# daviszhen/plan

Hardware: NVIDIA B200
Metric: tpch_q1_q6_q3_lineitem_rows_per_s (higher is better)
Workload: dtype int64 fixed-point (128-bit merge)

## Files before the change

### plan_b200/csrc/join.cu

```cuda
#include <algorithm>

#include <cub/device/device_scan.cuh>

#include "hostdec.hpp"
#include "join.cuh"
#include "exchange.cuh"
#include "leftcount.cuh"
#include "pipeline.hpp"

namespace pg {

namespace {

struct BaseCol { int slot = -1, col = -1; };

struct Stage {
    int src_slot = -1;
    std::vector<Range> ranges;
    bool has_probe = false;
    int probe_mode = 0;
    bool existence_only = false;
    int probe_key_col = -1;
    int probe_stage = -1;
    int ins_key_col = -1;
// ... 13 lines not shown
    bool no_table = false;
    i64 dup_keys = 0;
    bool bitmap_only() const { return jt.bitmap && !payload_needed && (dup_keys == 0 || existence_only); }
};

static u64 next_pow2(u64 x)
{
    u64 p = 1;
    while (p < x) p <<= 1;
    return p;
}

static TypedCol typed(const pg_table *t, int col)
{
    TypedCol c;
    c.p = t->cols[(size_t)col].d_data;
    c.width = t->cols[(size_t)col].phys_width();
    c.base = t->cols[(size_t)col].base;
    c.valid = t->cols[(size_t)col].has_nulls ? t->cols[(size_t)col].d_valid : nullptr;
    return c;
}

}

struct JoinAggPipeline : Pipeline {
    pg_plan *plan = nullptr;
    std::vector<std::unique_ptr<Stage>> stages;
    int src_slot = -1;
    std::vector<Range> ranges;
    int probe_key_col = -1;
    GroupSpec gs{};
    int nparts = 0;
    BaseCol part_col[GT_MAXKEYPARTS];
    int part_type[GT_MAXKEYPARTS] = {0, 0, 0};
    std::vector<AggExpr> aggs;
    std::vector<int> agg_scale;
    std::vector<int> agg_plane;
    bool no_join = false;
    int top_probe_mode = 0;
    int hav_plane = -1;
    i64 hav_lo = INT64_MIN, hav_hi = INT64_MAX;
    i64 group_hint = 0;
    i64 key_min = 0;
    u64 key_domain = 0;
    bool key_sorted = false;
    bool device_only = false;
    i64 dev_ngroups = 0;
    std::vector<Stage::Extra> extras;
    bool fd_mode = false;
    struct FdOut { int kind, slot, col, via_key_col, via_stage; };
    std::vector<FdOut> fd;
    int fd_stage = -1;
    int star_anchor = -1;
    bool star = false;
    int main_stage = -1;
    struct HRef { int origin = 0, col = -1; };
    struct HLookup { int nkey = 1; HRef key[2]; int stage = -1; };
    struct HPart { HRef v; int fn = 0; i64 lo = 0; int n = 1; int type = 0; };
    struct HTerm { int nfac = 0; HRef fac[3]; i64 fc[3] = {0, 0, 0}; int fs[3] = {1, 1, 1}; i64 mul = 1; };
    std::vector<HLookup> lookups;
    std::vector<int> origin_slot;
    std::vector<HPart> sparts;
    std::vector<HTerm> sterms;
    int star_ngroups = 0, star_scale = 0;
    i128 star_worst = 0;
    int xl = -1;
    std::vector<int> xcols;
    int x_term_mask[STAR_MAXTERM] = {0, 0};
    int x_fac_col[STAR_MAXTERM][3] = {{0, 0, 0}, {0, 0, 0}};
    DevBuf d_xb_rec, d_xb_dest, d_xb_send, d_xb_recv, d_xp_rec, d_xp_dest, d_xp_send, d_xp_recv;
    i64 xb_recv_rows = 0;
    EventPair ev_xb, ev_xp;
    i64 x_sent_rows = 0, x_sent_bytes = 0;
    DevBuf d_star, d_star_all;
    PinBuf h_star;
    Stage &top_stage_ref() { return *stages[(size_t)(main_stage >= 0 ? main_stage : (int)stages.size() - 1)]; }
    DevBuf d_edges, d_dense;
    int dense_passes = 0;
    std::vector<std::pair<int, int>> outs;
    std::vector<int> group_out_type;
    i64 algorithmic_bytes = 0, main_bytes = 0;
    DevBuf d_counters, d_gt, d_overflow, d_out_klo, d_out_khi, d_out_acc;
    u64 gt_cap = 0;
    i64 out_cap = 0;
    EventPair ev_all, ev_main;
    bool shuffle = false;
    bool gather_ranks = false;
    DevBuf d_g_klo, d_g_khi, d_g_acc, d_g_cnt;
    PinBuf h_out;
    static constexpr int SG_CAP = 256;
    DevBuf d_sg;
    PinBuf h_sg;
    bool has_topk = false;
    TopkKey topk_key{};
    i64 topk_limit = -1;
    DevBuf d_hist, d_cand_klo, d_cand_khi, d_cand_acc, d_tstate;
    PinBuf h_hist;
    i64 cand_cap = 0;

    int topk_preselect(i64 *ngroups, pg_result *res)
    {
        cudaStream_t st = ctx().stream;
        i64 n = *ngroups, k = topk_limit;
        if (k < 0 || n <= k) return PG_OK;
        if (k == 0) { *ngroups = 0; return PG_OK; }
        const int planes = gs.nacc + 1 + (int)fd.size();
// ... 127 lines not shown
    {
        unsigned long long h[8];
        PG_CUDA(cudaMemcpyAsync(h, d_counters.p, 64, cudaMemcpyDeviceToHost, ctx().stream));
        PG_CUDA(cudaStreamSynchronize(ctx().stream));
        memcpy(out2, h, 32);
        for (int idx = 0; idx < 2; idx++)
            if (((deferred_stats >> idx) & 1u) && cur_res) {
                cur_res->stats.aux[2 + 2 * idx] = (i64)h[4 + 2 * idx];
                cur_res->stats.aux[3 + 2 * idx] = (i64)h[5 + 2 * idx];
            }
        return PG_OK;
    }

    static int grid_rows(i64 nrows)
    {
        i64 g = (nrows + 255) / 256;
        i64 cap = (i64)ctx().prop.multiProcessorCount * 8;
        if (g > cap) g = cap;
        return (int)std::max<i64>(g, 1);
    }

    DevBuf d_hits, d_hit_count;
    static constexpr i64 HIT_CHUNK = (i64)1 << 30;

    static bool two_phase_ok(const PipeParams &pp, const pg_table *t, bool ins_sink)
    {
        bool any_valid = pp.probe_key.valid != nullptr || (ins_sink && pp.ins_key.valid != nullptr);
        for (int k = 0; k < pp.npred; k++) any_valid = any_valid || pp.pred[k].col.valid != nullptr;
        return (pp.has_probe ? pp.probe.bitmap != nullptr : ins_sink) && pp.nlike == 0 && pp.npred <= 1 && (pp.npred == 0 || !pp.pred[0].is_set) && !any_valid && t->nrows < ((i64)1 << 32) &&
               !getenv("PG_JOIN_GENERIC");
    }

    int launch_filter(PipeParams &pp, i64 lo, i64 hi)
    {
        cudaStream_t st = ctx().stream;
        if (!d_hit_count.p) PG_TRY(d_hit_count.alloc(8));
        size_t need = (size_t)std::max<i64>(hi - lo, 1) * 4;
        if (d_hits.bytes < need) PG_TRY(d_hits.alloc(need));
        PG_CUDA(cudaMemsetAsync(d_hit_count.p, 0, 8, st));
        pp.row_begin = lo;
        pp.row_end = hi;
        pp.hits = d_hits.as<unsigned>();
        pp.hit_count = d_hit_count.as<unsigned long long>();
        if (try_staged_filter(pp, lo, hi) == PG_OK) return PG_OK;
        i64 ntiles = (hi - lo + SA_TILE - 1) / SA_TILE;
        int grid = (int)std::max<i64>(std::min<i64>(ntiles, (i64)ctx().prop.multiProcessorCount * 8), 1);
        if (pp.npred == 1) filter_hits_kernel<true, 1><<<grid, SA_THREADS, 0, st>>>(pp);
        else filter_hits_kernel<false, 1><<<grid, SA_THREADS, 0, st>>>(pp);
        PG_CUDA(cudaGetLastError());
        return PG_OK;
    }

    bool staged_filter_used = false;
    int try_staged_filter(const PipeParams &pp, i64 lo, i64 hi)
    {
        if (getenv("PG_NO_STAGED") && atoi(getenv("PG_NO_STAGED"))) return PG_EUNSUPPORTED;
        if (hi <= lo || (lo & 15) != 0 || pp.npred > 1) return PG_EUNSUPPORTED;
        const TypedCol &kc = pp.probe_key;
        if (!kc.p || kc.width > 4 || kc.valid) return PG_EUNSUPPORTED;
        FilterSParams fp{};
        fp.bitmap = pp.has_probe ? pp.probe.bitmap : nullptr;
        if (pp.has_probe && !fp.bitmap) return PG_EUNSUPPORTED;
        fp.anti = pp.probe_mode == 2 ? 1 : 0;
        auto stored_span = [](const TypedCol &c, i64 *tmin, i64 *tmax) {
            if (c.width == 4) { *tmin = INT32_MIN; *tmax = INT32_MAX; }
            else { *tmin = 0; *tmax = c.width == 2 ? 0xffff : 0xff; }
        };
        if (fp.bitmap) {
            if (pp.probe.domain > 0xffffffffULL) return PG_EUNSUPPORTED;
            i64 tmin, tmax;
            stored_span(kc, &tmin, &tmax);
            const i128 delta = (i128)kc.base - (i128)pp.probe.bm_min;
            const i128 omin = (i128)tmin + delta, omax = (i128)tmax + delta;
            if (omax >= ((i128)1 << 32) || omin <= (i128)pp.probe.domain - ((i128)1 << 32)) return PG_EUNSUPPORTED;
            fp.kdelta = (unsigned)(u64)(i64)delta;
            fp.dom = (unsigned)pp.probe.domain;
        }
        fp.p_lo = 0; fp.p_span = 0xffffffffu;
        fp.st.ncol = 0;
        fp.rpw[0] = 0; fp.roff[0] = 0;
        int pi = -1;
        if (pp.npred == 1) {
            const TypedCol &pc = pp.pred[0].col;
            if (pp.pred[0].is_set || pc.width > 4 || pc.valid) return PG_EUNSUPPORTED;
            i64 tmin, tmax;
            stored_span(pc, &tmin, &tmax);
            i128 a = (i128)pp.pred[0].lo - pc.base, b = (i128)pp.pred[0].hi - pc.base;
            if (a < tmin) a = tmin;
            if (b > tmax) b = tmax;
            if (pp.pred[0].lo > pp.pred[0].hi || a > b) return PG_EUNSUPPORTED;
            fp.p_lo = (unsigned)(int32_t)(i64)a;
            fp.p_span = (unsigned)(u64)(i64)(b - a);
            pi = fp.st.ncol;
            fp.st.src[pi] = (const char *)pc.p + lo * pc.width;
            fp.st.pw[pi] = pc.width;
            fp.st.ncol++;
        }
        int ki = -1;
        if (pi >= 0 && fp.st.src[pi] == (const char *)kc.p + lo * kc.width) ki = pi;
        else {
            ki = fp.st.ncol;
            fp.st.src[ki] = (const char *)kc.p + lo * kc.width;
            fp.st.pw[ki] = kc.width;
            fp.st.ncol++;
        }
        const int qpt = 2;
        const int tile_rows = ST_CONS_WARPS * 128 * qpt;
        stage_layout(&fp.st, tile_rows);
        if (pi >= 0) { fp.rpw[0] = fp.st.pw[pi]; fp.roff[0] = fp.st.off[pi]; }
        fp.rpw[1] = fp.st.pw[ki]; fp.roff[1] = fp.st.off[ki];
        fp.st.nstage = getenv("PG_NSTAGE") ? atoi(getenv("PG_NSTAGE")) : 4;
        fp.row_begin = lo;
        fp.nloc = hi - lo;
        fp.hits = pp.hits;
        fp.hit_count = pp.hit_count;
        fp.counters = pp.counters;
        typedef void (*FK)(const FilterSParams);
        FK k;
        if (const char *m = getenv("PG_STAGED_FILTER_MASK")) {
            const int cls = (fp.rpw[0] == 2 && fp.rpw[1] == 4) ? 1 : (fp.rpw[0] == 0 && fp.rpw[1] == 4) ? 2 : fp.rpw[0] == 0 ? 4 : 8;
            if (!(atoi(m) & cls)) return PG_EUNSUPPORTED;
        }
        if (fp.rpw[0] == 2 && fp.rpw[1] == 4) k = filter_hits_staged_kernel<2, 4, 2>;
        else if (fp.rpw[0] == 0 && fp.rpw[1] == 4) k = filter_hits_staged_kernel<0, 4, 2>;
        else if (fp.rpw[0] == 0) k = filter_hits_staged_kernel<0, -1, 2>;
        else k = filter_hits_staged_kernel<-1, -1, 2>;
        const size_t smem = (size_t)ST_HDR + (size_t)fp.st.nstage * fp.st.stage_bytes;
        PG_CUDA(cudaFuncSetAttribute((const void *)k, cudaFuncAttributeMaxDynamicSharedMemorySize, (int)smem));
        int per_sm = 1;
        cudaOccupancyMaxActiveBlocksPerMultiprocessor(&per_sm, (const void *)k, ST_THREADS, smem);
        const i64 ntiles = (fp.nloc + tile_rows - 1) / tile_rows;
        const int grid = (int)std::max<i64>(1, std::min<i64>(ntiles, (i64)ctx().prop.multiProcessorCount * std::max(per_sm, 1)));
        k<<<grid, ST_THREADS, smem, ctx().stream>>>(fp);
        PG_CUDA(cudaGetLastError());
        staged_filter_used = true;
        return PG_OK;
    }

    template <int SINK>
    int launch_sink(const PipeParams &pp)
    {
        hits_sink_kernel<SINK><<<ctx().prop.multiProcessorCount * 8, 256, 0, ctx().stream>>>(pp);
        PG_CUDA(cudaGetLastError());
        return PG_OK;
    }

    template <int SINK>
    int launch_pipe(const PipeParams &pp, const pg_table *t)
    {
        pipeline_kernel<SINK><<<grid_rows(pp.pipe_hi > 0 ? pp.pipe_hi - pp.pipe_lo : t->nrows), 256, 0, ctx().stream>>>(pp);
        PG_CUDA(cudaGetLastError());
        return PG_OK;
    }

    int prepare_table(Stage &s, i64 nbuild, const Column &keycol)
    {
        cudaStream_t st = ctx().stream;
        u64 nb = next_pow2((u64)std::max<i64>((nbuild * 2 + HT_BUCKET - 1) / HT_BUCKET, 16));
        if (nbuild > s.capacity_rows || !s.d_slots.p) {
            PG_TRY(s.d_slots.alloc(nb * HT_BUCKET * sizeof(longlong2)));
            s.capacity_rows = (i64)(nb * HT_BUCKET / 2);
        } else {
            nb = next_pow2((u64)std::max<i64>((nbuild * 2 + HT_BUCKET - 1) / HT_BUCKET, 16));
        }
        PG_CUDA(cudaMemsetAsync(s.d_slots.p, 0x80, nb * HT_BUCKET * sizeof(longlong2), st));
        s.jt.slots = s.d_slots.as<longlong2>();
        s.jt.bucket_mask = nb - 1;
        {
            i128 dom = (i128)keycol.vmax - (i128)keycol.vmin + 1;
            int lg = 0;
            while (((u64)1 << lg) < nb) lg++;
            bool asc = keycol.stats_ok && keycol.adjacent_descents * 100 <= std::max<i64>(nbuild, 1) && dom > 0 && dom <= ((i128)1 << 34) && lg <= 29;
            if (getenv("PG_JOIN_ORDER_PRESERVING")) asc = asc && atoi(getenv("PG_JOIN_ORDER_PRESERVING")) != 0;
            if (s.ins_key_col2 >= 0) asc = false;
            s.jt.order_preserving = asc ? 1 : 0;
            s.jt.log2buckets = lg;
            s.jt.domain = dom > 0 ? (u64)dom : 1;
        }
        s.jt.rank_prefix = nullptr;
        s.jt.rank_payload = nullptr;
        s.jt.rank_identity = 0;
        s.rank_index = false;
        s.jt.bitmap = nullptr;
        s.jt.bm_min = keycol.vmin;
        s.jt.bm_max = keycol.vmax;
        i128 domain = (i128)keycol.vmax - (i128)keycol.vmin + 1;
        if (keycol.stats_ok && domain > 0 && domain <= ((i128)1 << 32) && s.ins_key_col2 < 0) {
// ... 629 lines not shown
                const AggExpr &a = aggs[(size_t)o.second];
                col.width = a.width;
                col.scale = a.scale;
                if (a.fn == PG_AGG_AVG && a.ltype == PG_LT_DOUBLE) {
                    col.type = PG_T_FLOAT64;
                    col.data.resize(live.size() * 8);
                    double *d = (double *)col.data.data();
                    for (size_t i = 0; i < live.size(); i++) {
                        const i128 v = sums[(size_t)live[i]];
                        if (v >= ((i128)1 << 53) || v <= -((i128)1 << 53)) PG_FAIL(PG_EOVERFLOW, "avg(INT): sum not exact in float64");
                        d[i] = (double)(i64)v / (double)cnts[(size_t)live[i]];
                    }
                } else if (a.fn == PG_AGG_AVG) {
                    col.type = PG_T_DECIMAL128;
                    col.data.resize(live.size() * sizeof(pg_decimal));
                    pg_decimal *d = (pg_decimal *)col.data.data();
                    for (size_t i = 0; i < live.size(); i++) {
                        HDec sd, nd, qd;
                        if (!hd_from_i128(sums[(size_t)live[i]], star_scale, &sd) || !hd_from_i128((i128)cnts[(size_t)live[i]], 0, &nd) || !hd_quo(sd, nd, &qd))
                            PG_FAIL(PG_EOVERFLOW, "avg: decimal division failed");
                        d[i].coef = qd.coef;
                        d[i].scale = qd.scale;
                        d[i].neg = qd.neg ? 1u : 0u;
                    }
                } else if (a.fn == PG_AGG_COUNT || a.ltype == PG_LT_HUGEINT) {
                    col.type = PG_T_HUGEINT;
                    col.data.resize(live.size() * sizeof(pg_hugeint));
                    pg_hugeint *d = (pg_hugeint *)col.data.data();
                    for (size_t i = 0; i < live.size(); i++) {
                        const i128 v = a.fn == PG_AGG_COUNT ? (i128)cnts[(size_t)live[i]] : sums[(size_t)live[i]];
                        d[i].lower = (u64)v;
                        d[i].upper = (i64)(v >> 64);
                    }
                } else {
                    col.type = PG_T_DECIMAL128;
                    col.data.resize(live.size() * sizeof(pg_decimal));
                    pg_decimal *d = (pg_decimal *)col.data.data();
                    for (size_t i = 0; i < live.size(); i++) {
                        const i128 v = sums[(size_t)live[i]];
                        const u128 m = v < 0 ? (u128)(-v) : (u128)v;
                        if (m >= (u128)10000000000000000000ULL) PG_FAIL(PG_EOVERFLOW, "star join: a group sum needs more than 19 digits");
                        d[i].neg = v < 0;
                        d[i].coef = (u64)m;
                        d[i].scale = star_scale;
                    }
                }
            }
            res->cols.push_back(std::move(col));
        }
        tr.mark("result columns");
        return PG_OK;
    }

    int run(pg_result *res) override
    {
        Context &c = ctx();
        cudaStream_t st = c.stream;
        PG_TRY(ev_all.init());
        PG_TRY(ev_main.init());
        Trace tr("joinagg");
        PG_CUDA(cudaEventRecord(ev_all.a, st));
        res->stats.kernel_launches = 0;
        cur_res = res;
        deferred_stats = 0;
        PG_CUDA(cudaMemsetAsync(d_counters.p, 0, 128, st));
        x_sent_rows = x_sent_bytes = 0;
        for (size_t i = 0; i < stages.size(); i++) {
            if (xl >= 0 && (int)i == lookups[(size_t)xl].stage) { PG_TRY(run_exchange_build(*stages[i], res)); tr.mark("build stage (row exchange)"); continue; }
            PG_TRY(run_build_stage(*stages[i], res, (int)i));
            tr.mark("build stage");
        }
        if (star) return run_star(res, tr);

        const pg_table *t = tab(src_slot);
        PipeParams pp{};
        pp.nrows = t->nrows;
        PG_TRY(fill_preds(pp, ranges, src_slot));
        pp.has_probe = no_join ? 0 : 1;
        if (!no_join) {
            Stage &last = top_stage_ref();
            pp.probe_key = typed(t, probe_key_col);
            pp.probe = last.jt;
            pp.probe_bitmap_only = last.bitmap_only() ? 1 : 0;
            pp.probe_mode = top_probe_mode;
        }
        PG_TRY(fill_extras(pp, extras, src_slot));
        pp.counters = d_counters.as<unsigned long long>();
        pp.gs = gs;
        u64 cap = next_pow2((u64)std::max<i64>((no_join ? group_hint : stages.back()->built_rows) * 2, 1024));
        unsigned long long cnt[4] = {0, 0, 0, 0};
        const bool two_phase = !no_join && two_phase_ok(pp, t, false);
        const bool single_filter = two_phase && t->nrows <= HIT_CHUNK;
        unsigned long long filter_pass = 0;
        if (single_filter) {
            PG_CUDA(cudaMemsetAsync(d_counters.p, 0, 32, st));
            PG_CUDA(cudaEventRecord(ev_main.a, st));
            PG_TRY(launch_filter(pp, 0, t->nrows));
            unsigned long long c0[4];
            PG_TRY(read_counters(c0));
            filter_pass = c0[0];
            const bool exact = pp.probe_bitmap_only || pp.probe_mode != 0 || stages.back()->dup_keys == 0 || stages.back()->unique_key;
            if (exact) cap = next_pow2((u64)std::max<i64>((i64)std::min<unsigned long long>(c0[3], (unsigned long long)cap / 2) * 2, 1024));
            res->stats.kernel_launches += 1;
            tr.mark("probe filter");
        }
        bool one_shape = false;
        if (no_join) {
            bool pred_valid = false;
            for (int k = 0; k < pp.npred; k++) pred_valid = pred_valid || pp.pred[k].col.valid != nullptr;
            one_shape = !pred_valid && gs.nparts == 1 && gs.nacc == 1 && gs.nfac[0] == 1 && pp.npred <= 1 &&
                        (pp.npred == 0 || !pp.pred[0].is_set) && !getenv("PG_GROUP_GENERIC");
        }
        const bool sorted_runs = one_shape && key_sorted && t->nrows > 0 && !(shuffle && c.world > 1) && !getenv("PG_NO_SORTED_RUNS");
        i64 ngroups = 0;
        if (sorted_runs) {
            constexpr int WPB = SA_THREADS / 32;
            const i64 ntiles = (t->nrows + RUN_WTILE - 1) / RUN_WTILE;
            i64 nwarps = std::max<i64>(std::min<i64>(ntiles, (i64)c.prop.multiProcessorCount * 4 * WPB), 1);
            const i64 chunk_tiles = (ntiles + nwarps - 1) / nwarps;
            nwarps = (ntiles + chunk_tiles - 1) / chunk_tiles;
            const i64 grid = (nwarps + WPB - 1) / WPB;
            const i64 nchunks = grid * WPB;
            if (d_edges.bytes < (size_t)nchunks * 2 * sizeof(RunEdge)) PG_TRY(d_edges.alloc((size_t)nchunks * 2 * sizeof(RunEdge)));
            RunEdge *first = d_edges.as<RunEdge>(), *last = first + nchunks;
            i64 want = hav_plane >= 0 ? std::max<i64>(t->nrows / 64, 1 << 16) : std::min<i64>(t->nrows, group_hint * 4);
            for (int attempt = 0;; attempt++) {
                if (want > out_cap) {
                    PG_TRY(d_out_klo.alloc((size_t)want * 8));
                    PG_TRY(d_out_khi.alloc((size_t)want * 8));
                    PG_TRY(d_out_acc.alloc((size_t)want * 8 * (size_t)(gs.nacc + 1)));
                    out_cap = want;
                }
                PG_CUDA(cudaMemsetAsync(d_counters.p, 0, 32, st));
                RunOut ro{d_out_klo.as<i64>(), d_out_khi.as<i64>(), d_out_acc.as<i64>(), out_cap, d_counters.as<unsigned long long>() + 2,
                          hav_plane, hav_lo, hav_hi};
                PG_CUDA(cudaEventRecord(ev_main.a, st));
                if (pp.npred == 1) run_group_kernel<true><<<(int)grid, SA_THREADS, 0, st>>>(pp, ro, first, last, chunk_tiles);
                else run_group_kernel<false><<<(int)grid, SA_THREADS, 0, st>>>(pp, ro, first, last, chunk_tiles);
                PG_CUDA(cudaGetLastError());
                run_fixup_kernel<<<(int)((nchunks + 255) / 256), 256, 0, st>>>(first, last, (int)nchunks, ro);
                PG_CUDA(cudaGetLastError());
                PG_CUDA(cudaEventRecord(ev_main.b, st));
                res->stats.kernel_launches += 2;
                PG_TRY(read_counters(cnt));
                ngroups = (i64)cnt[2];
// ... 294 lines not shown
                PG_CUDA(cudaMemcpyAsync(nh.p, d_out_khi.p, (size_t)ngroups * 8, cudaMemcpyDeviceToDevice, st));
                for (int a = 0; a < planes; a++)
                    PG_CUDA(cudaMemcpyAsync(na.as<i64>() + (size_t)a * (size_t)maxn, d_out_acc.as<i64>() + (size_t)a * (size_t)out_cap,
                                            (size_t)ngroups * 8, cudaMemcpyDeviceToDevice, st));
                PG_CUDA(cudaStreamSynchronize(st));
                std::swap(d_out_klo.p, nk.p); std::swap(d_out_klo.bytes, nk.bytes);
                std::swap(d_out_khi.p, nh.p); std::swap(d_out_khi.bytes, nh.bytes);
                std::swap(d_out_acc.p, na.p); std::swap(d_out_acc.bytes, na.bytes);
                out_cap = maxn;
            }
            size_t seg = (size_t)maxn * 8;
            if (d_g_klo.bytes < seg * (size_t)c.world) {
                PG_TRY(d_g_klo.alloc(seg * (size_t)c.world));
                PG_TRY(d_g_khi.alloc(seg * (size_t)c.world));
                PG_TRY(d_g_acc.alloc(seg * (size_t)c.world * (size_t)planes));
            }
            PG_TRY(comm_allgather(d_out_klo.p, d_g_klo.p, seg, st));
            PG_TRY(comm_allgather(d_out_khi.p, d_g_khi.p, seg, st));
            for (int a = 0; a < planes; a++)
                PG_TRY(comm_allgather(d_out_acc.as<i64>() + (size_t)a * (size_t)out_cap,
                                      (char *)d_g_acc.p + (size_t)a * seg * (size_t)c.world, seg, st));
            PG_TRY(host_arrays(total));
            i64 off = 0;
            for (int r = 0; r < c.world; r++) {
                size_t n = (size_t)counts[(size_t)r];
                if (n) {
                    PG_CUDA(cudaMemcpyAsync(h_klo + off, (char *)d_g_klo.p + seg * (size_t)r, n * 8, cudaMemcpyDeviceToHost, st));
                    PG_CUDA(cudaMemcpyAsync(h_khi + off, (char *)d_g_khi.p + seg * (size_t)r, n * 8, cudaMemcpyDeviceToHost, st));
                    for (int a = 0; a < planes; a++)
                        PG_CUDA(cudaMemcpyAsync(h_acc + (size_t)a * (size_t)total + (size_t)off,
                                                (char *)d_g_acc.p + (size_t)a * seg * (size_t)c.world + seg * (size_t)r, n * 8,
                                                cudaMemcpyDeviceToHost, st));
                }
                off += (i64)n;
            }
            ngroups = total;
        } else {
            PG_TRY(host_arrays(ngroups));
            if (ngroups > 0) {
                PG_CUDA(cudaMemcpyAsync(h_klo, d_out_klo.p, (size_t)ngroups * 8, cudaMemcpyDeviceToHost, st));
                PG_CUDA(cudaMemcpyAsync(h_khi, d_out_khi.p, (size_t)ngroups * 8, cudaMemcpyDeviceToHost, st));
                for (int a = 0; a < planes; a++)
                    PG_CUDA(cudaMemcpyAsync(h_acc + (size_t)a * (size_t)ngroups, d_out_acc.as<i64>() + (size_t)a * (size_t)out_cap,
                                            (size_t)ngroups * 8, cudaMemcpyDeviceToHost, st));
            }
        }
        PG_CUDA(cudaEventRecord(ev_all.b, st));
        PG_CUDA(cudaStreamSynchronize(st));
        tr.mark("gather+d2h");
        res->stats.kernel_ms = ev_all.ms();
        res->stats.main_kernel_ms = ev_main.ms();
        res->stats.rows_scanned = t->nrows;
        res->stats.algorithmic_bytes = algorithmic_bytes;
        res->stats.main_kernel_bytes = main_bytes + (i64)cnt[1] * 32 * (gs.nparts + 2 * gs.nacc);
        res->stats.aux[0] = (i64)cnt[0];
        res->stats.aux[1] = (i64)cnt[1];

        res->nrows = ngroups;
        for (auto &o : outs) {
            ResCol col;
            if (o.first == 0 && fd_mode) {
                const FdOut &fo = fd[(size_t)o.second];
                const Column &cc = tab(fo.slot)->cols[(size_t)fo.col];
                const i64 *src = h_acc + (size_t)(gs.nacc + 1 + o.second) * (size_t)ngroups;
                col.type = cc.type;
                col.width = cc.width;
                col.scale = cc.scale;
                if (cc.type == PG_T_DICT8) col.dict = cc.dict;
                const int w = type_size(cc.type);
                col.data.resize((size_t)ngroups * (size_t)w);
                if (cc.type == PG_T_VARCHAR) {
                    size_t total = 0;
                    for (i64 i = 0; i < ngroups; i++) {
                        if (src[i] < 0 || src[i] + 1 >= (i64)cc.h_off.size()) PG_FAIL(PG_ECUDA, "internal: dependent key row %lld out of range", (long long)src[i]);
                        total += (size_t)(cc.h_off[(size_t)src[i] + 1] - cc.h_off[(size_t)src[i]]);
                    }
                    col.heap.resize(total + 1);
                    pg_string *d = (pg_string *)col.data.data();
                    size_t at = 0;
                    for (i64 i = 0; i < ngroups; i++) {
                        const size_t b = (size_t)cc.h_off[(size_t)src[i]], n = (size_t)cc.h_off[(size_t)src[i] + 1] - b;
                        memcpy(col.heap.data() + at, cc.h_bytes.data() + b, n);
                        d[i].data = col.heap.data() + at;
                        d[i].len = (int64_t)n;
                        at += n;
                    }
                } else {
                    for (i64 i = 0; i < ngroups; i++) {
                        if (w == 8) ((i64 *)col.data.data())[i] = src[i];
                        else if (w == 4) ((int32_t *)col.data.data())[i] = (int32_t)src[i];
                        else col.data[(size_t)i] = (uint8_t)src[i];
                    }
                }
            } else if (o.first == 0) {
                int k = o.second;
                col.type = group_out_type[(size_t)k];
                const int w = type_size(col.type);
                col.data.resize((size_t)ngroups * (size_t)w);
                if (k == 0 && w == 8) {
                    if (ngroups) memcpy(col.data.data(), h_klo, (size_t)ngroups * 8);
                } else if (k == 0) {
                    int32_t *d = (int32_t *)col.data.data();
                    for (i64 i = 0; i < ngroups; i++) d[i] = (int32_t)h_klo[i];
                } else if (w == 4) {
                    int32_t *d = (int32_t *)col.data.data();
                    if (k == 1) for (i64 i = 0; i < ngroups; i++) d[i] = (int32_t)(h_khi[i] >> 32);
                    else for (i64 i = 0; i < ngroups; i++) d[i] = (int32_t)(h_khi[i] & 0xffffffffLL);
// ... 966 lines not shown
            p->shuffle = !(ok && disjoint);
            if (p->fd_mode) {
                if (bt->dist == PG_DIST_REPLICATED) PG_FAIL(PG_EUNSUPPORTED, "dependent group keys over a replicated build table and a sharded probe");
                for (auto &f : p->fd)
                    if (p->tab(f.slot)->cols[(size_t)f.col].type == PG_T_VARCHAR && p->tab(f.slot)->dist != PG_DIST_REPLICATED)
                        PG_FAIL(PG_EUNSUPPORTED, "VARCHAR group key from a sharded table");
                p->shuffle = false;
            }
        }
    }
    if (plan->topk && !plan->topk->order.empty() && !nested && !p->fd_mode) {
        auto o = aggn.outs[(size_t)plan->topk->order[0].first];
        TopkKey tk{};
        tk.desc = plan->topk->order[0].second ? 1 : 0;
        tk.div = 1;
        if (o.first == 0) {
            tk.src = o.second;
        } else {
            if (aggn.aggs[(size_t)o.second].fn == PG_AGG_AVG) goto no_device_topk;
            tk.src = 3;
            tk.plane = p->agg_plane[(size_t)o.second];
            int sc = p->agg_scale[(size_t)o.second];
            for (int i = 2; i < sc; i++) tk.div *= 10;
        }
        p->has_topk = true;
        p->topk_key = tk;
        p->topk_limit = plan->topk->limit;
    }
no_device_topk:
    PG_TRY(p->d_counters.alloc(128));
    PG_TRY(p->d_overflow.alloc(4));
    std::string ex = "JoinAgg[inner hash join chain -> global group table] stages:";
    for (auto &sp : p->stages) {
        char b[256];
        snprintf(b, sizeof b, " build(%s%s key=%s%s%s)", sp->sub ? "aggregate over " : "", p->tab(sp->src_slot)->name.c_str(),
                 p->tab(sp->src_slot)->cols[(size_t)sp->ins_key_col].name.c_str(), sp->has_probe ? " probing previous" : "",
                 sp->extras.empty() ? "" : " +existence tests");
        ex += b;
    }
    if (p->fd_mode) ex += " group-by=build row id (dependent keys fetched per group)";
    char b[320];
    if (p->no_join)
        snprintf(b, sizeof b, "GroupBy[global open-addressing table] scan(%s) kernel=pipeline_kernel<SINK_GROUP> group_keys=%d sums=%d%s%s%s",
                 st->name.c_str(), p->nparts, p->gs.nacc, p->hav_plane >= 0 ? " having" : "",
                 p->key_sorted ? " sorted-run reduce-by-key when the shape allows (run_group_kernel)"
                               : (p->key_domain > 0 && p->key_domain <= ((u64)1 << 28)) ? " dense direct-addressed accumulators in L2-sized key slices when the shape allows (group1_dense_kernel)" : "",
                 p->shuffle ? " exchange=all-to-all(hash-partitioned)" : "");
    else
        snprintf(b, sizeof b, " probe(%s key=%s) kernel=filter_hits_kernel+hits_sink_kernel<SINK_GROUP> group_keys=%d sums=%d%s", st->name.c_str(),
                 st->cols[(size_t)p->probe_key_col].name.c_str(), p->nparts, p->gs.nacc,
                 p->shuffle ? " exchange=all-to-all(hash-partitioned)" : "");
    if (p->no_join) ex = b; else ex += b;
    p->explain = ex;
    *out = std::move(p);
    return PG_OK;
}

}


namespace pg {

namespace {

struct LeftCountPipeline : Pipeline {
    JoinAggPipeline jp;
    int anchor_col = -1;
    int build_slot = -1, build_key_col = -1;
    int arg_col = -1;
    bool null_if_empty = false;
    bool outer = false;
    std::vector<Range> build_ranges;
    std::vector<std::pair<int, int>> outs;
    LcFilter fa{}, fb{};
    DevBuf d_counts, d_cnt, d_hist, d_out_key, d_out_cnt;
    i64 big_cap = 0;
    EventPair ev_all, ev_main;
    i64 main_bytes = 0, algorithmic_bytes = 0;

    int fill(LcFilter &f, const std::vector<Range> &rs, int slot, std::vector<std::string> *desc)
    {
        const pg_table *t = jp.tab(slot);
        const bool bytewise = getenv("PG_LIKE_BYTEWISE") && atoi(getenv("PG_LIKE_BYTEWISE")) != 0;
        f.npred = f.nlike = 0;
        for (auto &r : rs) {
            if (!r.like) {
                if (f.npred >= PIPE_MAXPRED) PG_FAIL(PG_EUNSUPPORTED, "more than %d predicate columns on one scan", PIPE_MAXPRED);
                SrcPred &q = f.pred[f.npred++];
                q.col = typed(t, r.col);
                q.lo = r.lo;
                q.hi = r.hi;
                q.is_set = r.is_set ? 1 : 0;
                memcpy(q.mask, r.set, sizeof q.mask);
                continue;
            }
            const Column &col = t->cols[(size_t)r.col];
            if (!col.d_off) PG_FAIL(PG_EUNSUPPORTED, "string predicate on %s without a device copy of the text", col.name.c_str());
            if (f.nlike >= GEN_MAXLIKE) PG_FAIL(PG_EUNSUPPORTED, "more than %d string predicates on one scan", GEN_MAXLIKE);
            GenLike &l = f.like[f.nlike++];
            memset(&l, 0, sizeof l);
            l.bytes = col.d_bytes;
            l.off = (const i64 *)col.d_off;
            std::vector<std::string> segs;
            if (r.like <= 2 && !bytewise && like_segments(r.pat, &segs)) {
                l.kind = r.like == 1 ? GEN_LIKE_WORDS : GEN_NOTLIKE_WORDS;
                l.plen = (int)segs.size();
// ... 280 lines not shown
```

### plan_b200/csrc/join.cuh

```cuda
#pragma once
#include "common.cuh"
#include "scanagg.cuh"

namespace pg {

constexpr i64 HT_EMPTY = (i64)0x8080808080808080ULL;
constexpr int HT_BUCKET = 4;

__host__ __device__ __forceinline__ u64 mix64(u64 x)
{
    x ^= x >> 33; x *= 0xff51afd7ed558ccdULL; x ^= x >> 33; x *= 0xc4ceb9fe1a85ec53ULL; x ^= x >> 33;
    return x;
}

struct JoinTable {
    longlong2 *slots;
    u64 bucket_mask;
    unsigned *bitmap;
    i64 bm_min, bm_max;
    unsigned long long *dups;
    int order_preserving;
    int log2buckets;
    u64 domain;
    const unsigned *rank_prefix;
// ... 843 lines not shown
        base = __shfl_sync(0xffffffffu, base, 0);
        for (int i = lane; i < nbuf; i += 32) p.hits[base + i] = s_buf[warp][i];
        __syncwarp();
        n_hits += lane == 0 ? (unsigned)nbuf : 0u;
        nbuf = 0;
    }
    int pos = nbuf + incl - c;
#pragma unroll
    for (int q = 0; q < QPT; q++) {
        const unsigned rowid = (unsigned)(p.row_begin + row0) + (unsigned)((warp * QPT + q) * 128 + lane * 4);
#pragma unroll
        for (int j = 0; j < 4; j++)
            if (hitmask & (1u << (4 * q + j))) s_buf[warp][pos++] = rowid + j;
    }
    nbuf += total;
    __syncwarp();
}

template <int WP, int WK, int QPT>
__global__ void __launch_bounds__(ST_THREADS)
filter_hits_staged_kernel(const FilterSParams p)
{
    extern __shared__ __align__(128) unsigned char st_smem[];
    __shared__ unsigned s_buf[ST_CONS_WARPS][512];
    const StageDesc &d = p.st;
    const StageRing ring = stage_ring_init(st_smem, d);
    const i64 ntiles = (p.nloc + d.tile_rows - 1) / d.tile_rows;
    const TileSeq seq = tile_seq(ntiles, 0);
    const int warp = threadIdx.x >> 5, lane = threadIdx.x & 31;
    if (warp == ST_CONS_WARPS) {
        stage_produce(ring, d, seq);
        return;
    }
    StageCursor cur = {0, 0};
    int nbuf = 0;
    unsigned n_pass = 0, n_hits = 0;
    const bool partial = last_tile_is_partial(seq, ntiles, p.nloc, d.tile_rows);
    const int nwhole = (int)seq.count - (partial ? 1 : 0);
    for (int k = 0; k < nwhole; k++)
        filter_tile<WP, WK, QPT, false>(p, ring, cur, warp, lane, seq.first + (i64)k * seq.step, s_buf, nbuf, n_pass, n_hits);
    if (partial) filter_tile<WP, WK, QPT, true>(p, ring, cur, warp, lane, ntiles - 1, s_buf, nbuf, n_pass, n_hits);
    if (nbuf) {
        unsigned long long base = 0;
        if (lane == 0) base = atomicAdd(p.hit_count, (unsigned long long)nbuf);
        base = __shfl_sync(0xffffffffu, base, 0);
        for (int i = lane; i < nbuf; i += 32) p.hits[base + i] = s_buf[warp][i];
        n_hits += lane == 0 ? (unsigned)nbuf : 0u;
    }
    unsigned long long np = (unsigned long long)warp_sum((i64)n_pass), nh = (unsigned long long)warp_sum((i64)n_hits);
    if (lane == 0 && np) atomicAdd(&p.counters[0], np);
    if (lane == 0 && nh) atomicAdd(&p.counters[3], nh);
}

template <int SINK>
__global__ void __launch_bounds__(256)
hits_sink_kernel(const PipeParams p)
{
    const unsigned long long n = *p.hit_count;
    unsigned long long n_join = 0;
    for (unsigned long long i = (unsigned long long)blockIdx.x * blockDim.x + threadIdx.x; i < n; i += (unsigned long long)gridDim.x * blockDim.x) {
        const i64 row = (i64)p.hits[i];
        if (p.nextra && !extras_pass(p, row)) continue;
        auto sink = [&](u64 build_row) {
            n_join++;
            if (SINK == SINK_INSERT) {
                i64 key = load_typed(p.ins_key, row);
                if (p.ins_key2.p) key = (key << 32) | (load_typed(p.ins_key2, row) & 0xffffffffLL);
                jt_insert(p.ins, key, (u64)row);
            } else if (SINK == SINK_BITMAP) {
                u64 off = (u64)(load_typed(p.ins_key, row) - p.ins.bm_min);
                atomicOr(p.ins.bitmap + (off >> 5), 1u << (off & 31));
            } else if (SINK == SINK_GROUP) {
                auto val = [&](const ValRef &r) { return r.from_build == 2 ? (i64)build_row : load_typed(r.col, r.from_build ? (i64)build_row : row); };
                i64 klo = val(p.gs.part[0]);
                i64 khi = 0;
                if (p.gs.nparts > 1) khi = val(p.gs.part[1]) << 32;
                if (p.gs.nparts > 2) khi |= val(p.gs.part[2]) & 0xffffffffLL;
                i64 vals[GT_MAXACC];
                for (int a = 0; a < p.gs.nacc; a++) {
                    i64 x = 1;
                    for (int f = 0; f < p.gs.nfac[a]; f++) x *= p.gs.fc[a][f] + p.gs.fs[a][f] * val(p.gs.fac[a][f]);
                    vals[a] = x;
                }
                gt_update(p.gt, klo, khi, vals);
            }
        };
        if (!p.has_probe || p.probe_bitmap_only || p.probe_mode != 0) sink(0);
        else jt_probe(p.probe, load_typed(p.probe_key, row), sink);
    }
    n_join = (unsigned long long)warp_sum((i64)n_join);
    if ((threadIdx.x & 31) == 0 && n_join) atomicAdd(&p.counters[1], n_join);
}

constexpr int STAR_MAXLOOKUP = 5, STAR_MAXTERM = 2, STAR_MAXPART = 2, STAR_MAXGROUPS = 4096;
struct StarLookup {
    int nkey;
    ValRef key[2];
    JoinTable jt;
    int existence;
};
struct StarPart {
    ValRef v;
    int fn;
    i64 lo;
    int n;
};
// ... 494 lines not shown
```

Baseline: 393.0 billion.

## Fuse probe filter with rank-indexed accumulation for unique-key join aggregates

Adds a path for join-aggregates whose group keys come from a unique-key build table. It fuses the staged probe filter with per-rank atomic accumulation of the sums, then compacts the non-empty ranks into the output. This replaces the separate hit-list, sink and hash-group-by passes. The cost is atomic contention on popular ranks and a dense accumulator array sized by the number of build rows.

After: 343.9 billion, median of 6. -12.5%, worse.

```diff
diff --git a/plan_b200/csrc/join.cu b/plan_b200/csrc/join.cu
--- a/plan_b200/csrc/join.cu
+++ b/plan_b200/csrc/join.cu
@@ -89,6 +89,11 @@
     std::vector<FdOut> fd;
     int fd_stage = -1;
     int star_anchor = -1;
+    bool row_acc = false;
+    RankKeys acc_keys{};
+    std::string explain_table, explain_acc;
+    DevBuf d_racc;
+    bool row_acc_ran = false;
     bool star = false;
     int main_stage = -1;
     struct HRef { int origin = 0, col = -1; };
@@ -322,13 +327,13 @@
     }
 
     bool staged_filter_used = false;
-    int try_staged_filter(const PipeParams &pp, i64 lo, i64 hi)
+    static int staged_filter_params(const PipeParams &pp, i64 lo, i64 hi, FilterSParams &fp)
     {
         if (getenv("PG_NO_STAGED") && atoi(getenv("PG_NO_STAGED"))) return PG_EUNSUPPORTED;
         if (hi <= lo || (lo & 15) != 0 || pp.npred > 1) return PG_EUNSUPPORTED;
         const TypedCol &kc = pp.probe_key;
         if (!kc.p || kc.width > 4 || kc.valid) return PG_EUNSUPPORTED;
-        FilterSParams fp{};
+        fp = FilterSParams{};
         fp.bitmap = pp.has_probe ? pp.probe.bitmap : nullptr;
         if (pp.has_probe && !fp.bitmap) return PG_EUNSUPPORTED;
         fp.anti = pp.probe_mode == 2 ? 1 : 0;
@@ -385,6 +390,27 @@
         fp.hits = pp.hits;
         fp.hit_count = pp.hit_count;
         fp.counters = pp.counters;
+        return PG_OK;
+    }
+
+    template <typename P>
+    static int launch_staged(void (*k)(const P), const P &prm, const FilterSParams &fp)
+    {
+        const size_t smem = (size_t)ST_HDR + (size_t)fp.st.nstage * fp.st.stage_bytes;
+        PG_CUDA(cudaFuncSetAttribute((const void *)k, cudaFuncAttributeMaxDynamicSharedMemorySize, (int)smem));
+        int per_sm = 1;
+        cudaOccupancyMaxActiveBlocksPerMultiprocessor(&per_sm, (const void *)k, ST_THREADS, smem);
+        const i64 ntiles = (fp.nloc + fp.st.tile_rows - 1) / fp.st.tile_rows;
+        const int grid = (int)std::max<i64>(1, std::min<i64>(ntiles, (i64)ctx().prop.multiProcessorCount * std::max(per_sm, 1)));
+        k<<<grid, ST_THREADS, smem, ctx().stream>>>(prm);
+        PG_CUDA(cudaGetLastError());
+        return PG_OK;
+    }
+
+    int try_staged_filter(const PipeParams &pp, i64 lo, i64 hi)
+    {
+        FilterSParams fp;
+        if (staged_filter_params(pp, lo, hi, fp) != PG_OK) return PG_EUNSUPPORTED;
         typedef void (*FK)(const FilterSParams);
         FK k;
         if (const char *m = getenv("PG_STAGED_FILTER_MASK")) {
@@ -395,14 +421,7 @@
         else if (fp.rpw[0] == 0 && fp.rpw[1] == 4) k = filter_hits_staged_kernel<0, 4, 2>;
         else if (fp.rpw[0] == 0) k = filter_hits_staged_kernel<0, -1, 2>;
         else k = filter_hits_staged_kernel<-1, -1, 2>;
-        const size_t smem = (size_t)ST_HDR + (size_t)fp.st.nstage * fp.st.stage_bytes;
-        PG_CUDA(cudaFuncSetAttribute((const void *)k, cudaFuncAttributeMaxDynamicSharedMemorySize, (int)smem));
-        int per_sm = 1;
-        cudaOccupancyMaxActiveBlocksPerMultiprocessor(&per_sm, (const void *)k, ST_THREADS, smem);
-        const i64 ntiles = (fp.nloc + tile_rows - 1) / tile_rows;
-        const int grid = (int)std::max<i64>(1, std::min<i64>(ntiles, (i64)ctx().prop.multiProcessorCount * std::max(per_sm, 1)));
-        k<<<grid, ST_THREADS, smem, ctx().stream>>>(fp);
-        PG_CUDA(cudaGetLastError());
+        PG_TRY(launch_staged(k, fp, fp));
         staged_filter_used = true;
         return PG_OK;
     }
@@ -1138,6 +1157,57 @@
         return PG_OK;
     }
 
+    int run_rank_acc(const PipeParams &pp, const pg_table *t, pg_result *res, Trace &tr, bool *ran)
+    {
+        Context &c = ctx();
+        cudaStream_t st = c.stream;
+        *ran = false;
+        const Stage &top = *stages.back();
+        if (!top.rank_index || top.jt.rank_identity || !top.jt.rank_payload || (shuffle && c.world > 1)) return PG_OK;
+        FilterSParams fp;
+        if (staged_filter_params(pp, 0, t->nrows, fp) != PG_OK) return PG_OK;
+        void (*k)(const RankAccParams);
+        if (fp.rpw[0] == 2 && fp.rpw[1] == 4) k = filter_rankacc_staged_kernel<2, 4, 2>;
+        else if (fp.rpw[0] == 0 && fp.rpw[1] == 4) k = filter_rankacc_staged_kernel<0, 4, 2>;
+        else return PG_OK;
+        *ran = true;
+        const u64 nranks = (u64)std::max<i64>(top.built_rows, 0);
+        const int nacc = gs.nacc;
+        const size_t acc_bytes = (size_t)std::max<u64>(nranks, 1) * (8 * (size_t)nacc + 4);
+        if (d_racc.bytes < acc_bytes) PG_TRY(d_racc.alloc(acc_bytes));
+        RankAccParams rp{};
+        rp.f = fp;
+        rp.jt = top.jt;
+        rp.gs = gs;
+        for (int a = 0; a < gs.nacc; a++) for (int f = 0; f < gs.nfac[a]; f++) rp.need_build |= gs.fac[a][f].from_build;
+        rp.acc = d_racc.as<unsigned long long>();
+        rp.cnt = (unsigned *)(rp.acc + (size_t)nranks * (size_t)nacc);
+        rp.nranks = nranks;
+        PG_CUDA(cudaMemsetAsync(d_racc.p, 0, (size_t)nranks * (8 * (size_t)nacc + 4), st));
+        PG_CUDA(cudaMemsetAsync(d_counters.p, 0, 32, st));
+        PG_CUDA(cudaEventRecord(ev_main.a, st));
+        PG_TRY(launch_staged(k, rp, fp));
+        PG_CUDA(cudaEventRecord(ev_main.b, st));
+        tr.mark("probe filter + rank accumulate");
+        const i64 want = (i64)std::max<u64>(nranks, 1);
+        if (want > out_cap) {
+            PG_TRY(d_out_klo.alloc((size_t)want * 8));
+            PG_TRY(d_out_khi.alloc((size_t)want * 8));
+            PG_TRY(d_out_acc.alloc((size_t)want * 8 * (size_t)(nacc + 1)));
+            out_cap = want;
+        }
+        if (nranks > 0)
+            rank_compact_kernel<<<(int)std::min<u64>((nranks + 255) / 256, (u64)c.prop.multiProcessorCount * 8), 256, 0, st>>>(
+                rp.acc, rp.cnt, nranks, top.jt.rank_payload, acc_keys, d_out_klo.as<i64>(), d_out_khi.as<i64>(), d_out_acc.as<i64>(), out_cap,
+                d_counters.as<unsigned long long>() + 2);
+        PG_CUDA(cudaGetLastError());
+        res->stats.kernel_launches += 2;
+        unsigned long long cnt[4];
+        PG_TRY(read_counters(cnt));
+        row_acc_ran = true;
+        return finish_groups((i64)cnt[2], cnt, res, tr);
+    }
+
     int run(pg_result *res) override
     {
         Context &c = ctx();
@@ -1177,6 +1247,13 @@
         unsigned long long cnt[4] = {0, 0, 0, 0};
         const bool two_phase = !no_join && two_phase_ok(pp, t, false);
         const bool single_filter = two_phase && t->nrows <= HIT_CHUNK;
+        row_acc_ran = false;
+        if (row_acc) {
+            bool ran = false;
+            if (single_filter && !getenv("PG_JOIN_NO_ROW_ACC")) PG_TRY(run_rank_acc(pp, t, res, tr, &ran));
+            explain = ran ? explain_acc : explain_table;
+            if (ran) return PG_OK;
+        }
         unsigned long long filter_pass = 0;
         if (single_filter) {
             PG_CUDA(cudaMemsetAsync(d_counters.p, 0, 32, st));
@@ -1577,7 +1654,12 @@
         res->stats.main_kernel_ms = ev_main.ms();
         res->stats.rows_scanned = t->nrows;
         res->stats.algorithmic_bytes = algorithmic_bytes;
-        res->stats.main_kernel_bytes = main_bytes + (i64)cnt[1] * 32 * (gs.nparts + 2 * gs.nacc);
+        int gathered = gs.nparts + 2 * gs.nacc;
+        if (row_acc_ran) {
+            gathered = 0;
+            for (int a = 0; a < gs.nacc; a++) gathered += gs.nfac[a];
+        }
+        res->stats.main_kernel_bytes = main_bytes + (i64)cnt[1] * 32 * gathered;
         res->stats.aux[0] = (i64)cnt[0];
         res->stats.aux[1] = (i64)cnt[1];
 
@@ -2650,6 +2732,30 @@
                  p->shuffle ? " exchange=all-to-all(hash-partitioned)" : "");
     if (p->no_join) ex = b; else ex += b;
     p->explain = ex;
+    if (!p->no_join && p->top_probe_mode == 0 && !p->fd_mode && p->hav_plane < 0 && p->extras.empty() && st->total_rows() < ((i64)1 << 32)) {
+        const Stage &T = *p->stages[(size_t)top_stage];
+        bool ok = T.unique_key && !T.sub && top_stage + 1 == (int)p->stages.size();
+        RankKeys rk{};
+        rk.nparts = p->nparts;
+        rk.nacc = p->gs.nacc;
+        for (int k = 0; k < p->nparts && ok; k++) {
+            BaseCol bc;
+            const Expr *ge = strip_value_preserving_casts(&aggn.groups[(size_t)k]);
+            if (!resolve(top, ge->idx, &bc)) ok = false;
+            else if (bc.slot == build_slot) rk.part[k] = typed(bt, bc.col);
+            else if (bc.slot == p->src_slot && bc.col == p->probe_key_col) rk.part[k] = typed(bt, T.ins_key_col);
+            else ok = false;
+        }
+        if (ok) {
+            p->row_acc = true;
+            p->acc_keys = rk;
+            p->explain_table = ex;
+            snprintf(b, sizeof b, " probe(%s key=%s) kernel=filter_rankacc_staged_kernel (groups=ranks of %s) group_keys=%d sums=%d", st->name.c_str(),
+                     st->cols[(size_t)p->probe_key_col].name.c_str(), bt->name.c_str(), p->nparts, p->gs.nacc);
+            p->explain_acc = "JoinAgg[inner hash join chain -> rank-indexed accumulators]" + ex.substr(ex.find(" stages:"), ex.find(" probe(") - ex.find(" stages:")) + b;
+            p->explain = p->explain_acc;
+        }
+    }
     *out = std::move(p);
     return PG_OK;
 }
diff --git a/plan_b200/csrc/join.cuh b/plan_b200/csrc/join.cuh
--- a/plan_b200/csrc/join.cuh
+++ b/plan_b200/csrc/join.cuh
@@ -919,6 +919,133 @@
     if (lane == 0 && nh) atomicAdd(&p.counters[3], nh);
 }
 
+struct RankAccParams {
+    FilterSParams f;
+    JoinTable jt;
+    GroupSpec gs;
+    int need_build;
+    unsigned long long *acc;
+    unsigned *cnt;
+    u64 nranks;
+};
+
+template <int WP, int WK, int QPT, bool MASK>
+__device__ __forceinline__ void rankacc_tile(const RankAccParams &p, const StageRing &ring, StageCursor &cur, int warp, int lane, i64 tile,
+                                             unsigned &n_pass, unsigned &n_join)
+{
+    const FilterSParams &fp = p.f;
+    const char *stg = stage_acquire(ring, fp.st, cur);
+    Quad<WP> dv[QPT];
+    Quad<WK> kv[QPT];
+#pragma unroll
+    for (int q = 0; q < QPT; q++) {
+        const int qrow = (warp * QPT + q) * 128 + lane * 4;
+        dv[q].load(stg + fp.roff[0], qrow, fp.rpw[0]);
+        kv[q].load(stg + fp.roff[1], qrow, fp.rpw[1]);
+    }
+    stage_release(ring, fp.st, cur);
+    const unsigned *__restrict__ bm = fp.bitmap;
+    const i64 row0 = tile * fp.st.tile_rows;
+    const int rows_in_tile = MASK ? (int)(fp.nloc - row0) : 0;
+    bool ok[QPT][4];
+    unsigned w[QPT][4], off[QPT][4];
+#pragma unroll
+    for (int q = 0; q < QPT; q++) {
+        const int rem = rows_in_tile - ((warp * QPT + q) * 128 + lane * 4);
+        auto row = [&](auto jc) {
+            constexpr int J = decltype(jc)::v;
+            ok[q][J] = (!MASK || J < rem) && (WP == 0 || (dv[q].template get<J>() - fp.p_lo) <= fp.p_span);
+            off[q][J] = kv[q].template get<J>() + fp.kdelta;
+            w[q][J] = ok[q][J] && off[q][J] < fp.dom ? __ldg(bm + (off[q][J] >> 5)) : 0u;
+        };
+        PG_FOR4(row);
+    }
+    unsigned hitmask = 0;
+#pragma unroll
+    for (int q = 0; q < QPT; q++)
+#pragma unroll
+        for (int j = 0; j < 4; j++) {
+            n_pass += ok[q][j] ? 1u : 0u;
+            if (ok[q][j] && ((w[q][j] >> (off[q][j] & 31u)) & 1u)) hitmask |= 1u << (4 * q + j);
+        }
+#pragma unroll
+    for (int q = 0; q < QPT; q++)
+#pragma unroll
+        for (int j = 0; j < 4; j++) {
+            if (!(hitmask & (1u << (4 * q + j)))) continue;
+            n_join++;
+            const i64 row = fp.row_begin + row0 + (warp * QPT + q) * 128 + lane * 4 + j;
+            bool set;
+            const unsigned r = jt_rank(p.jt, off[q][j], &set);
+            const i64 brow = p.need_build ? (i64)__ldg(p.jt.rank_payload + r) : 0;
+            for (int a = 0; a < p.gs.nacc; a++) {
+                i64 x = 1;
+                for (int f = 0; f < p.gs.nfac[a]; f++) x *= p.gs.fc[a][f] + p.gs.fs[a][f] * load_typed(p.gs.fac[a][f].col, p.gs.fac[a][f].from_build ? brow : row);
+                atomicAdd(p.acc + (u64)a * p.nranks + r, (unsigned long long)x);
+            }
+            atomicAdd(p.cnt + r, 1u);
+        }
+}
+
+template <int WP, int WK, int QPT>
+__global__ void __launch_bounds__(ST_THREADS)
+filter_rankacc_staged_kernel(const RankAccParams p)
+{
+    extern __shared__ __align__(128) unsigned char st_smem[];
+    const StageDesc &d = p.f.st;
+    const StageRing ring = stage_ring_init(st_smem, d);
+    const i64 ntiles = (p.f.nloc + d.tile_rows - 1) / d.tile_rows;
+    const TileSeq seq = tile_seq(ntiles, 0);
+    const int warp = threadIdx.x >> 5, lane = threadIdx.x & 31;
+    if (warp == ST_CONS_WARPS) {
+        stage_produce(ring, d, seq);
+        return;
+    }
+    StageCursor cur = {0, 0};
+    unsigned n_pass = 0, n_join = 0;
+    const bool partial = last_tile_is_partial(seq, ntiles, p.f.nloc, d.tile_rows);
+    const int nwhole = (int)seq.count - (partial ? 1 : 0);
+    for (int k = 0; k < nwhole; k++)
+        rankacc_tile<WP, WK, QPT, false>(p, ring, cur, warp, lane, seq.first + (i64)k * seq.step, n_pass, n_join);
+    if (partial) rankacc_tile<WP, WK, QPT, true>(p, ring, cur, warp, lane, ntiles - 1, n_pass, n_join);
+    unsigned long long np = (unsigned long long)warp_sum((i64)n_pass), nj = (unsigned long long)warp_sum((i64)n_join);
+    if (lane == 0 && np) atomicAdd(&p.f.counters[0], np);
+    if (lane == 0 && nj) atomicAdd(&p.f.counters[1], nj);
+}
+
+struct RankKeys {
+    int nparts, nacc;
+    TypedCol part[GT_MAXKEYPARTS];
+};
+
+static __global__ void __launch_bounds__(256)
+rank_compact_kernel(const unsigned long long *__restrict__ acc, const unsigned *__restrict__ cnt, u64 nranks, const unsigned *__restrict__ payload,
+                    const RankKeys k, i64 *__restrict__ out_klo, i64 *__restrict__ out_khi, i64 *__restrict__ out_acc, i64 max_out,
+                    unsigned long long *__restrict__ counter)
+{
+    const int lane = threadIdx.x & 31;
+    for (u64 i0 = ((u64)blockIdx.x * blockDim.x + threadIdx.x) - lane; i0 < nranks; i0 += (u64)gridDim.x * blockDim.x) {
+        const u64 i = i0 + lane;
+        const unsigned c = i < nranks ? cnt[i] : 0u;
+        const unsigned m = __ballot_sync(0xffffffffu, c != 0);
+        if (!m) continue;
+        unsigned long long base = 0;
+        if (lane == 0) base = atomicAdd(counter, (unsigned long long)__popc(m));
+        base = __shfl_sync(0xffffffffu, base, 0);
+        if (c == 0) continue;
+        const unsigned long long o = base + __popc(m & ((1u << lane) - 1u));
+        if ((i64)o >= max_out) continue;
+        const i64 brow = (i64)payload[i];
+        i64 khi = 0;
+        if (k.nparts > 1) khi = load_typed(k.part[1], brow) << 32;
+        if (k.nparts > 2) khi |= load_typed(k.part[2], brow) & 0xffffffffLL;
+        out_klo[o] = load_typed(k.part[0], brow);
+        out_khi[o] = khi;
+        for (int a = 0; a < k.nacc; a++) out_acc[(u64)a * (u64)max_out + o] = (i64)acc[(u64)a * nranks + i];
+        out_acc[(u64)k.nacc * (u64)max_out + o] = (i64)c;
+    }
+}
+
 template <int SINK>
 __global__ void __launch_bounds__(256)
 hits_sink_kernel(const PipeParams p)
```
